# emrullahArkun/tinycarlo

Measured on AMD Instinct MI355X. Metric: env-steps/sec (whole node), higher is better.
Workload: dtype f64; 1 GPU; cfg3: 4096 envs/GPU, simple_layout map, 64x64 'classes' obs, with camera laneline raster; envs_per_gpu=4096, steps_per_launch=128, entry_point=tc_step_multi, observations=every step's frame stored to its own row of a [128, N, ...] rollout buffer, preroll_steps=1024, calls_prepared=True, actions=v~U(0.3,1) s~U(-1,1) maneuver~U{0..3}/64 steps, on device, autoreset=True, spawn=host queue (reference seed parity), resets_since_queue_top_up=18375, max_respawns_of_one_env_since_top_up=11, spawn_queue_len=64, max_segments_per_frame=49, frames_sampled=196608, on_road_term=False, lds_bytes_per_env=9760

## Files before the change

### tinycarlo_amd/csrc/k_camera.h

```cpp
#ifndef K_CAMERA_H
#define K_CAMERA_H

#include "k_common.h"
#include "tc_clip.h"
#include "tc_cull.h"
#include "tc_pack.h"
#include "tc_device.h"

template <int K>
struct MapCache {
  double2 nd[K];
  int2 ed[K];
};

template <int K>
__device__ inline void cache_nodes(MapCache<K>& c, const DevMap& m, int base, int end, int tid) {
#pragma unroll
  for (int k = 0; k < K; k++) {
    const int i = base + k * TC_NT + tid;
    c.nd[k] = i < end ? m.nodes[i] : make_double2(0.0, 0.0);
  }
}
template <int K>
__device__ inline void cache_nodes_from(MapCache<K>& c, const double2* nodes, int base, int end, int tid) {
// ... 385 lines not shown
        }
      }
    }
  }
  __syncthreads();
  cam_chain_replay(Px, Py, Pz, flg, bit, tz, list, *cnt, 0.0, false, tid);
  __syncthreads();
}

struct FramePose {
  double x, y, cth, sth;
};

#define TC_POSE_ROW 16
#define TC_POSE_EMPTY 0xFFFFFFFFFFFFFFFFull
#define TC_FRAME_SKIPPED (-2)
__device__ __forceinline__ void cam_pose12(const KArgs& a, int cam_row, const FramePose& fp, double* pose) {
  double Ec[12];
  if (a.cam_E) {
#pragma unroll
    for (int i = 0; i < 12; i++) Ec[i] = a.cam_E[(size_t)cam_row * 12 + i];
  } else {
    const __attribute__((address_space(4))) double* ee = (const __attribute__((address_space(4))) double*)(unsigned long long)a.cam.E;
#pragma unroll
    for (int i = 0; i < 12; i++) Ec[i] = ee[i];
  }
  const double cth = fp.cth, sth = fp.sth;
  double R[16] = {cth, -sth, 0, 0, sth, cth, 0, 0, 0, 0, 1, 0, 0, 0, 0, 1};
  double Tm[16] = {1, 0, 0, -fp.x, 0, 1, 0, -fp.y, 0, 0, 1, 0, 0, 0, 0, 1};
  double car3d[16];
  d_matmul<4, 4, 4>(R, Tm, car3d);
  d_matmul<3, 4, 4>(Ec, car3d, pose);
}

#ifdef TC_ABLATE
__device__ unsigned long long tc_cull_counts[2];
#endif
__device__ __forceinline__ bool cam_cull(const KArgs& a, const double* pose) {
  typedef const __attribute__((address_space(4))) double* DConst;
  typedef const __attribute__((address_space(4))) int* IConst;
  typedef const __attribute__((address_space(4))) unsigned int* UConst;
  static_assert(offsetof(TcCullHead, margin) == 32 && offsetof(TcCullHead, nx) == 48 && offsetof(TcCullHead, n_special) == 56 &&
                    offsetof(TcCullHead, special) == 64 && TC_CULL_HEAD_BYTES % 4 == 0,
                "the fields are read by offset below");
  const DConst hd = (DConst)(unsigned long long)a.cull_tab;
  const IConst hi = (IConst)(unsigned long long)a.cull_tab;
  TcCullHead h;
  h.x0 = hd[0];
  h.y0 = hd[1];
  h.inv = hd[2];
  h.cell = hd[3];
  h.margin = hd[4];
  h.nx = hi[12];
  h.ny = hi[13];
  h.n_special = hi[14];
  int cell[TC_CULL_NC];
  unsigned int word[TC_CULL_NC];
#pragma unroll
  for (int i = 0; i < TC_CULL_NC; i++) {
    double wx, wy;
    tc_cull_world(pose, a.cull.c[i], &wx, &wy);
    cell[i] = uni_i(tc_cull_cell(h, wx, wy, a.cull.r[i]));
    word[i] = ((UConst)(unsigned long long)a.cull_tab)[(TC_CULL_HEAD_BYTES + (cell[i] > 0 ? cell[i] : 0)) >> 2];
  }
  bool empty = true;
#pragma unroll
  for (int i = 0; i < TC_CULL_NC; i++) {
    const int q = (int)((word[i] >> (8 * (cell[i] & 3))) & 255u);
    empty = empty && (cell[i] == TC_CULL_CELL_CLEAR || (cell[i] >= 0 && tc_cull_free(h, q, a.cull.r[i])));
  }
// ... 1 lines not shown
    const double mr = a.cull.max_range;
    for (int i = 0; i < h.n_special; i++) {
      const double z = __builtin_fma(pose[9], hd[9 + 2 * i], __builtin_fma(pose[8], hd[8 + 2 * i], pose[11]));
      empty = empty && tc_fabs(z + mr) >= TC_CULL_GUARD;
    }
  }
#ifdef TC_ABLATE
  if (threadIdx.x == 0) {
    atomicAdd(&tc_cull_counts[0], 1ull);
    if (empty) atomicAdd(&tc_cull_counts[1], 1ull);
  }
#endif
  return empty;
}

template <int K, bool LEAN = false>
__device__ __forceinline__ void cam_body(const KArgs& a, unsigned char* smem, int env, int cam_row, const double* pose_in, MapCache<K>& mc,
                                         const bool mc_loaded, const int tid, const int seg_row, int& nseg_out,
                                         unsigned int& used_out, const bool store_n = true) {
  unsigned int my_layers = 0;
  const DevMap& m = a.m;
  const int nwin_n = (m.total_nodes + TC_NT * K - 1) / (TC_NT * K), nwin_e = (m.total_edges + TC_NT * K - 1) / (TC_NT * K);
  const bool single = a.n_grp == 1 && !a.cam_nodes && a.grp_layer[0] == 0 && a.grp_layer[1] == m.C && nwin_n <= 1 && nwin_e <= 1;
  double pose[12];
#pragma unroll
  for (int i = 0; i < 12; i++) pose[i] = uni_d(pose_in[i]);
  if (a.frame_cull && cam_cull(a, pose)) {
    nseg_out = 0;
    used_out = 0;
    if (store_n && tid == 0) a.seg_n[(size_t)seg_row * a.N + env] = 0;
    return;
  }
  if (single && !mc_loaded) {
    cache_nodes(mc, m, 0, m.total_nodes, tid);
    cache_edges(mc, m, 0, m.total_edges, 0, tid);
  }
  double* Px = (double*)(smem + a.lds.off_p);
  double* Py = Px + a.cap_nodes;
  double* Pz = Py + a.cap_nodes;
  unsigned char* flg = smem + a.lds.off_flg;
  int* list = (int*)(smem + a.lds.off_list);
  int* cnt = (int*)(smem + a.lds.off_cnt);
  const DevCam& cam = a.cam;
  double Kc[9];
  if constexpr (LEAN) {
  } else if (a.cam_K) {
#pragma unroll
    for (int i = 0; i < 9; i++) Kc[i] = a.cam_K[(size_t)cam_row * 9 + i];
  } else {
    const __attribute__((address_space(4))) double* kk = (const __attribute__((address_space(4))) double*)(unsigned long long)cam.K;
#pragma unroll
    for (int i = 0; i < 9; i++) Kc[i] = kk[i];
  }
  int* seg_cnt = cnt + 5;
  const size_t seg_slot = (size_t)seg_row * a.N + env;
  int* segg = a.seg_g + seg_slot * a.seg_cap * 5;
  int nseg = 0;
  for (int g = 0; g < a.n_grp; g++) {
    const int l0 = a.grp_l0[g], l1 = a.grp_l1[g];
    const int gn0 = a.grp_n0[g], ge0 = a.grp_e0[g];
    const int nn = a.grp_n0[g + 1] - gn0, ne = a.grp_e0[g + 1] - ge0;
    const int nwn = (nn + TC_NT * K - 1) / (TC_NT * K), nwe = (ne + TC_NT * K - 1) / (TC_NT * K);
    const bool one = nwn <= 1 && nwe <= 1;
    const bool reload = !one;
    if (one && !single) {
      if (a.cam_nodes) {
        cache_nodes_from(mc, a.cam_nodes, gn0, gn0 + nn, tid);
        cache_edges_from(mc, a.cam_edges_g, ge0, ge0 + ne, gn0, tid);
      } else {
        cache_nodes(mc, m, gn0, gn0 + nn, tid);
        cache_edges(mc, m, ge0, ge0 + ne, gn0, tid);
      }
// ... 106 lines not shown
```

### tinycarlo_amd/csrc/k_common.h

```cpp
#ifndef K_COMMON_H
#define K_COMMON_H

#include <hip/hip_runtime.h>

#include "../../include/tinycarlo_hip.h"
#include "k_probe.h"
#include "tc_cull.h"
#include "tc_device.h"

#if defined(TC_PART) && defined(TC_DEV_FAST)
#error "the development builds are one translation unit"
#endif
#if defined(TC_PART) && TC_PART > 0
#define TC_PLAIN_KERNEL static
#else
#define TC_PLAIN_KERNEL
#endif

#define TC_PROF_RING 64
#define TC_RING_SLOTS 3
#define MODE_STEP 0
#define MODE_RESET 1
#define MODE_RENDER 2

// ... 75 lines not shown
  int* term_counters;
  int n_grp;
  int grp_layer[TC_MAX_GROUPS + 1];
  int grp_n0[TC_MAX_GROUPS + 1], grp_e0[TC_MAX_GROUPS + 1];
  int grp_l0[TC_MAX_GROUPS], grp_l1[TC_MAX_GROUPS];
  const double2* cam_nodes;
  const int2* cam_edges_g;
  int cap_nodes;
  const int* spawn_tab;
  int spawn_n;
  unsigned long long spawn_seed;
  unsigned int dbg;
  int seg_lds_off, seg_lds_cap;
  int clip_merge;
  int frame_cull;
  const unsigned char* cull_tab;
  TcCullCover cull;
};

__device__ __forceinline__ double d_readlane(double v, int l) {
  const int lo = __builtin_amdgcn_readlane(__double2loint(v), l);
  const int hi = __builtin_amdgcn_readlane(__double2hiint(v), l);
  return __hiloint2double(hi, lo);
}

__device__ __forceinline__ int uni_i(int v) { return __builtin_amdgcn_readfirstlane(v); }
__device__ __forceinline__ double uni_d(double v) {
  const int lo = __builtin_amdgcn_readfirstlane(__double2loint(v));
  const int hi = __builtin_amdgcn_readfirstlane(__double2hiint(v));
  return __hiloint2double(hi, lo);
// ... 56 lines not shown
```

### tinycarlo_amd/csrc/k_env.h

```cpp
#ifndef K_ENV_H
#define K_ENV_H

#include "k_camera.h"
#include "k_raster.h"
#include "k_sim.h"

struct StepArgs {
  KArgs a;
  RArgs r;
  MultiArgs ma;
  int mode, cdtype;
  unsigned int flags;
  const void* car_control;
  const int* maneuver;
  const int* spawn_nodes;
  const unsigned char* mask;
  const int* env_order;
  CarRows cr;
  EpArgs ep;
  CtrlArgs ct;
  CamBank cb;
  DriveArgs dr;
};

// ... 52 lines not shown
    MapCache<K> mc = {};
    FramePose fp;
    int cam_row;
    const bool need_b = k == nsteps - 1 || (sa.flags & TC_FI_INFO_EVERY) != 0;
    sim_body<K, FEAT>(sa.a, smem, env, sa.mode, (const char*)sa.car_control + row0 * 2 * esz, sa.cdtype, sa.maneuver + row0,
                         sa.spawn_nodes, sa.mask, sa.flags, roll_at(sa.ma.roll, row0, sa.a.m.C), tid, mc, fp, cam_row, need_b,
                         need_b || (CAM && sa.ma.cam_here), sa.cr, sa.ep, sa.ct, sa.cb, sa.dr);
    if (sa.ma.pose_rows) {
      double pose[12];
      cam_pose12(sa.a, cam_row, fp, pose);
      if (tid == 0) {
        double2* o = (double2*)(step_args().ma.pose_rows + (row0 + env) * TC_POSE_ROW);
#pragma unroll
        for (int i = 0; i < 6; i++) o[i] = make_double2(pose[2 * i], pose[2 * i + 1]);
        if (sa.flags & TC_FI_CAM_BANK) ((long long*)o)[12] = cam_row;
      }
    }
    if (CAM && sa.ma.cam_here) {
      if (wants_frame(sa)) {
        int nseg;
        unsigned int used;
        double pose[12];
        cam_pose12(sa.a, cam_row, fp, pose);
        cam_body<K>(sa.a, smem, env, cam_row, pose, mc, sa.mode != MODE_RENDER, tid, seg_row, nseg, used);
      }
      else if (tid == 0)
        step_args().a.seg_n[(size_t)seg_row * sa.a.N + env] = 0;
    }
    lds_sync();
  }
// ... 19 lines not shown
```

### tinycarlo_amd/csrc/k_envg.h

```cpp
#ifndef K_ENVG_H
#define K_ENVG_H

#include "k_env.h"

#define TC_EL 8
#ifndef TC_ENVG_NT
#define TC_ENVG_NT 256
#endif
#ifndef TC_ENVG_PRIO
#define TC_ENVG_PRIO 3
#endif
struct GroupLds {
  double dist[TC_MAX_LAYERS];
  int cnt[TC_MAX_TERMS];
};

typedef const __attribute__((address_space(3))) double* LdsDouble;
template <unsigned FEAT>
__device__ __forceinline__ void envg_kernel_body() {
  constexpr bool PER = (FEAT & TC_FEAT_CAR) != 0, EP = (FEAT & TC_FEAT_EP) != 0, CTRL = (FEAT & TC_FEAT_CTRL) != 0;
  __shared__ GroupLds glds[TC_ENVG_NT / TC_EL];
  extern __shared__ __align__(16) unsigned char gsm[];
  __builtin_amdgcn_s_setprio(TC_ENVG_PRIO);
  const StepArgs& s0 = step_args();
// ... 172 lines not shown
    if (sa.ma.pose_rows) {
      FramePose fp;
      fp.x = s.x;
      fp.y = s.y;
      fp.cth = have_trig ? s.cth : tc_cos(-s.theta);
      fp.sth = have_trig ? -s.sth : tc_sin(-s.theta);
      double pose[12];
      cam_pose12(sa.a, cam_row, fp, pose);
      if (live && sub == 0) {
        if (sa.ma.resident) {
          unsigned long long* o = (unsigned long long*)(sa.ma.pose_rows + (row0 + env) * TC_POSE_ROW);
#pragma unroll
          for (int i = 0; i < 12; i++)
            __hip_atomic_store(o + i, (unsigned long long)__double_as_longlong(pose[i]), __ATOMIC_RELAXED, __HIP_MEMORY_SCOPE_AGENT);
          if (bank) __hip_atomic_store(o + 12, (unsigned long long)(unsigned int)cam_row, __ATOMIC_RELAXED, __HIP_MEMORY_SCOPE_AGENT);
        } else {
          double2* o = (double2*)(sa.ma.pose_rows + (row0 + env) * TC_POSE_ROW);
#pragma unroll
          for (int i = 0; i < 6; i++) o[i] = make_double2(pose[2 * i], pose[2 * i + 1]);
          if (bank) ((long long*)o)[12] = cam_row;
        }
      }
    }
    if (track) {
      if (fat_lds) {
        trunc = d_find_local_path<TC_EL>(m, fl, s, track_man, status, pinfo, sub);
      } else {
        const FatGlobal fg = {m.lp_fat, m.lp_nodes};
        trunc = d_find_local_path<TC_EL>(m, fg, s, track_man, status, pinfo, sub);
      }
    }
    TSTAMP(27);
    const bool have_info = !fresh && s.lp_len >= 2;
    cte = 0;
    he = 0;
// ... 210 lines not shown
```

### tinycarlo_amd/csrc/k_frame.h

```cpp
#ifndef K_FRAME_H
#define K_FRAME_H

#include "k_camera.h"
#include "k_env.h"
#include "k_raster.h"
#include "k_sim.h"

struct FrameArgs {
  KArgs a;
  RArgs r;
  const double* pose_rows;
  const int* order;
  int gate;
  int bank;
  int recover_rows;
  unsigned int* abort_word;
  unsigned int* resident;
  long long gate_ticks;
  int gate_test;
};
typedef const __attribute__((address_space(4))) FrameArgs* FrameArgsConst;
__device__ __forceinline__ const FrameArgs& frame_args() {
  unsigned long long p = (unsigned long long)__builtin_amdgcn_kernarg_segment_ptr();
  asm volatile("" : "+s"(p));
  return *(const FrameArgs*)(FrameArgsConst)p;
}
__device__ __forceinline__ bool frame_pose(const size_t slot0, const int env, const int row, const bool wait, double* pose, int& cam_row) {
  const FrameArgs& fa = frame_args();
  const int tid = threadIdx.x;
  const int gate = fa.gate, bank = fa.bank;
  const int np = bank ? 13 : 12;
  cam_row = env;
  if (gate) {
    unsigned long long* prow = (unsigned long long*)(fa.pose_rows + (slot0 + env) * TC_POSE_ROW);
    unsigned long long v = 0;
    bool give_up = wait && fa.gate == 1 && fa.gate_test > 0 && (row + env) % fa.gate_test == 0;
    long long t0 = 0;
    while (!give_up) {
      v = tid < np ? __hip_atomic_load(prow + tid, __ATOMIC_RELAXED, __HIP_MEMORY_SCOPE_AGENT) : 0ull;
      if (__ballot(v == TC_POSE_EMPTY) == 0 || fa.gate == 2 || !wait) break;
      const long long now = wall_clock64();
      if (t0 == 0) t0 = now;
      if (now - t0 > fa.gate_ticks || __hip_atomic_load(fa.abort_word, __ATOMIC_RELAXED, __HIP_MEMORY_SCOPE_AGENT) != 0u)
        give_up = true;
      else
        __builtin_amdgcn_s_sleep(8);
    }
    if (give_up) {
      if (tid == 0) {
        if (t0 != 0) __hip_atomic_store(fa.abort_word, 1u, __ATOMIC_RELAXED, __HIP_MEMORY_SCOPE_AGENT);
        fa.a.seg_n[slot0 + env] = TC_FRAME_SKIPPED;
      }
      return false;
    }
    const unsigned int vlo = (unsigned int)v, vhi = (unsigned int)(v >> 32);
#pragma unroll
    for (int i = 0; i < 12; i++) {
      const unsigned long long q = (unsigned long long)(unsigned int)__builtin_amdgcn_readlane((int)vlo, i) |
                                   ((unsigned long long)(unsigned int)__builtin_amdgcn_readlane((int)vhi, i) << 32);
      pose[i] = __longlong_as_double((long long)q);
    }
    if (bank) {
      const unsigned int idx = (unsigned int)__builtin_amdgcn_readlane((int)vlo, 12);
      cam_row = (int)(idx < (unsigned int)bank ? idx : (unsigned int)bank - 1u);
    }
  } else {
    const __attribute__((address_space(4))) double* pr =
        (const __attribute__((address_space(4))) double*)(unsigned long long)(fa.pose_rows + (slot0 + env) * TC_POSE_ROW);
#pragma unroll
    for (int i = 0; i < 12; i++) pose[i] = pr[i];
    if (bank) {
      const unsigned int idx = ((const __attribute__((address_space(4))) unsigned int*)(unsigned long long)pr)[24];
      cam_row = (int)(idx < (unsigned int)bank ? idx : (unsigned int)bank - 1u);
    }
  }
  return true;
}

#ifndef TC_FRAME_WAVES_K5
#define TC_FRAME_WAVES_K5 5
#endif
#define TC_FRAME_WAVES(K, RBT) ((K) <= 5 ? ((RBT) == 32 ? TC_FRAME_WAVES_K5 : 4) : (K) <= 9 ? 3 : 2)
#define TC_FRAME_LEAN(K, RBT) ((K) <= 5 && (RBT) == 32)
template <int K, bool THICK, int FMT, bool HOT, int RBT, bool ONE_BAND = false>
__device__ __forceinline__ void frame_one(unsigned char* smem, const int env, const int rowy) {
  const int tid = threadIdx.x;
  int nseg;
  unsigned int used;
  {
    const FrameArgs& fa = frame_args();
    const int row = fa.r.seg_row0 + rowy;
    const size_t slot0 = (size_t)row * fa.a.N;
    double pose[12];
    int cam_row;
    if (!frame_pose(slot0, env, row, true, pose, cam_row)) return;
    MapCache<K> mc;
    TSTAMP_CLEAR();
    TSTAMP(3);
    TSTAMP_REAL(30);
    cam_body<K, TC_FRAME_LEAN(K, RBT)>(fa.a, smem, env, cam_row, pose, mc, false, tid, row, nseg, used, false);
  }
  const FrameArgs& fr = frame_args();
  const size_t slot0 = (size_t)(fr.r.seg_row0 + rowy) * fr.a.N;
  if (__builtin_expect(nseg > fr.a.seg_lds_cap, 0)) {
    if (HOT) {
      lds_sync();
      const LdsIntPtr sl = (LdsIntPtr)(smem + fr.a.seg_lds_off);
      int* sg = fr.a.seg_g + (slot0 + env) * fr.a.seg_cap * 5;
      for (int i = tid; i < 5 * fr.a.seg_lds_cap; i += TC_NT) sg[i] = sl[i];
    }
    __syncthreads();
  } else {
    lds_sync();
  }
  raster_body<THICK, FMT, HOT, RBT, TC_FRAME_LEAN(K, RBT), ONE_BAND>(fr.r, smem, env, fr.r.obs + (size_t)rowy * fr.r.obs_row_stride, tid, slot0, nseg, used,
                                           fr.r.noise_row0 + rowy);
  {
    const FrameArgs& fe = frame_args();
    const size_t slot = (size_t)(fe.r.seg_row0 + rowy) * fe.a.N + env;
    if (tid == 0) fe.a.seg_n[slot] = nseg;
    if (fe.gate && tid < (fe.bank ? 13 : 12))
      __hip_atomic_store((unsigned long long*)(fe.pose_rows + slot * TC_POSE_ROW) + tid, TC_POSE_EMPTY, __ATOMIC_RELAXED,
                         __HIP_MEMORY_SCOPE_AGENT);
  }
  TSTAMP_DUMP(env);
}

template <int K, bool THICK, int FMT, int RBT = RB_OF_K(K)>
__global__ __launch_bounds__(TC_NT, TC_FRAME_WAVES(K, RBT)) void tc_frame_kernel(FrameArgs fa_unused) {
  extern __shared__ __align__(16) unsigned char smem[];
  const FrameArgs& fa = frame_args();
  if ((int)blockIdx.x >= fa.a.N) return;
  const int env = fa.order ? uni_i(((const __attribute__((address_space(4))) int*)(unsigned long long)fa.order)[blockIdx.x])
                           : fa.a.env0 + (int)blockIdx.x;
  frame_one<K, THICK, FMT, true, RBT, TC_FRAME_LEAN(K, RBT)>(smem, env, (int)blockIdx.y);
}
// ... 103 lines not shown
```

### tinycarlo_amd/csrc/tc_cull.h

```cpp
#ifndef TC_CULL_H
#define TC_CULL_H
#include "tc_trig.h"

#ifndef TC_CULL_NC
#define TC_CULL_NC 2
#endif
#define TC_CULL_MAX_SPECIAL 16
#define TC_CULL_SLACK 1e-4
#define TC_CULL_GUARD 1e-6
#define TC_CULL_MAX_COORD 1e4
#define TC_CULL_MAX_CELLS (1 << 18)

struct TcCullHead {
  double x0, y0, inv, cell;
  double margin;
  double lmax;
  int nx, ny;
  int n_special, pad;
  double special[TC_CULL_MAX_SPECIAL][2];
};
#define TC_CULL_HEAD_BYTES 320
static_assert(sizeof(TcCullHead) <= TC_CULL_HEAD_BYTES, "the cells start TC_CULL_HEAD_BYTES into the buffer");

struct TcCullCover {
// ... 25 lines not shown
    const double z = __builtin_fma(pose[9], h.special[i][1], __builtin_fma(pose[8], h.special[i][0], pose[11]));
    ok &= tc_fabs(z + max_range) >= TC_CULL_GUARD;
  }
  return ok;
}
TC_HD int tc_cull_empty(const TcCullHead& h, const unsigned char* cells, const TcCullCover& cv, const double* pose) {
  if (!cv.on || h.nx <= 0) return 0;
  for (int i = 0; i < TC_CULL_NC; i++) {
    double wx, wy;
    tc_cull_world(pose, cv.c[i], &wx, &wy);
    const int cell = tc_cull_cell(h, wx, wy, cv.r[i]);
    if (cell == TC_CULL_CELL_MAYBE) return 0;
    if (cell >= 0 && !tc_cull_free(h, cells[cell], cv.r[i])) return 0;
  }
  return tc_cull_guard(h, pose, cv.max_range);
}

#include <math.h>
#include <vector>

static inline double tc_cull_seg_dist(double px, double py, double ax, double ay, double bx, double by) {
  const double ex = bx - ax, ey = by - ay, l2 = ex * ex + ey * ey;
  double t = l2 > 0 ? ((px - ax) * ex + (py - ay) * ey) / l2 : 0.0;
  t = t < 0 ? 0 : (t > 1 ? 1 : t);
  const double dx = px - (ax + t * ex), dy = py - (ay + t * ey);
  return sqrt(dx * dx + dy * dy);
}

static inline void tc_cull_plan(const double* nodes, int n_nodes, const int* edges, int n_edges, double cell, double margin,
                                std::vector<unsigned char>& out) {
// ... 213 lines not shown
```

### tinycarlo_amd/csrc/tinycarlo_hip.hip

```cpp
#include <hip/hip_runtime.h>
#include <math.h>
#include <stdio.h>
#include <stdlib.h>
#include <string.h>

#include <string>
#include <type_traits>
#include <vector>

#include "../../include/tinycarlo_hip.h"
#include "tc_device.h"
#include "tc_rng.h"
#include "tc_ctrl.h"
#include "tc_clip.h"
#include "tc_cull.h"

#include "k_probe.h"
#include "k_common.h"
#include "k_feat.h"
#include "k_collect.h"
#include "k_history.h"
#include "k_camera.h"
#include "k_sim.h"
#include "k_raster.h"
// ... 103 lines not shown
  if (feat & TC_FEAT_CTRL)
    return lift([](auto kc, auto t, auto f, auto ft) -> step_kern_t { return tc_drive_step_kernel<StepKRb<kc>::K, t, f, StepKRb<kc>::RB, ft>; },
                Kcodes{kcode}, Thicks{thick}, Fmts{fmt}, DriveFeats{feat});
  return lift([](auto kc, auto t, auto f, auto ft) -> step_kern_t { return tc_step_kernel<StepKRb<kc>::K, t, f, StepKRb<kc>::RB, ft>; },
              Kcodes{kcode}, Thicks{thick}, Fmts{fmt}, Feats{feat});
}
static step_kern_t env_kernel_of(int kv, bool cam, unsigned feat) {
  if (feat & TC_FEAT_CTRL)
    return lift([](auto k, auto c, auto ft) -> step_kern_t { return tc_drive_env_kernel<k, c, ft>; }, Kvars{kv}, Bools{cam}, DriveFeats{feat});
  return lift([](auto k, auto c, auto ft) -> step_kern_t { return tc_env_kernel<k, c, ft>; }, Kvars{kv}, Bools{cam}, Feats{feat});
}
static step_kern_t envg_kernel_of(unsigned feat) {
  if (feat & TC_FEAT_CTRL) return lift([](auto ft) -> step_kern_t { return tc_drive_envg_kernel<ft>; }, DriveFeats{feat});
  return lift([](auto ft) -> step_kern_t { return tc_envg_kernel<ft>; }, Feats{feat});
}
static frame_kern_t frame_kernel_of(int kcode, bool thick, int fmt, bool recover, bool banded) {
  return lift(
      [](auto kc, auto t, auto f, auto rec, auto bd) -> frame_kern_t {
        constexpr int K = FrameKRb<kc>::K, RB = FrameKRb<kc>::RB;
        if constexpr (rec) return tc_frame_recover_kernel<K, t, f, RB>;
        else if constexpr (bd && TC_FRAME_LEAN(K, RB)) return tc_frame_banded<K, t, f, RB>;
        else return tc_frame_kernel<K, t, f, RB>;
      },
      Kcodes{kcode}, Thicks{thick}, FrameFmts{fmt}, Bools{recover}, Bools{banded});
}
static int frame_k_of(int kcode) {
  return lift([](auto kc) -> int { return FrameKRb<kc>::K; }, Kcodes{kcode});
}
static int frame_rb_of(int kcode) {
  return lift([](auto kc) -> int { return FrameKRb<kc>::RB; }, Kcodes{kcode});
}
static raster_kern_t raster_kernel_of(bool thick, int fmt) {
  return lift([](auto t, auto f) -> raster_kern_t { return tc_raster_kernel<t, f>; }, Thicks{thick}, FrameFmts{fmt});
}

#endif

#if defined(TC_PART) && TC_PART == 1
TC_INST_PART1(template)
// ... 694 lines not shown
    const hipError_t he = rc == TC_OK ? hipFuncSetAttribute(kernel, hipFuncAttributeMaxDynamicSharedMemorySize, bytes) : hipSuccess;
    if (he == hipSuccess) return;
    (void)hipGetLastError();
    set_err(std::string("tc_env_create: cannot raise the dynamic LDS limit of ") + family + " to " + std::to_string(bytes) +
            " bytes: " + hipGetErrorString(he));
    rc = TC_E_HIP;
  };
  int lds = total > e->r_lds ? total : e->r_lds;
  if (e->frame_lds > lds) lds = e->frame_lds;
  if (lds > 48 * 1024)
    for (int kcode : {516, 5, 8, 9})
      for (int t = 0; t < 2; t++)
        for (int fmt : {TC_FMT_CLASSES, TC_FMT_CLASSES_BITS, TC_FMT_RGB}) {
          for (unsigned feat = 0; feat <= (TC_FEAT_CTRL | TC_FEAT_ALL) && fmt != TC_FMT_CLASSES_BITS; feat++)
            raise((const void*)step_kernel_of(kcode, t, fmt, feat), lds, (feat & TC_FEAT_CTRL) ? "tc_drive_step_kernel" : "tc_step_kernel");
          for (int banded = 0; banded < 2; banded++)
            raise((const void*)frame_kernel_of(kcode, t, fmt, false, banded), lds, "tc_frame_kernel");
        }
  const size_t envg_lds = ((size_t)m.total_edges * 48 + 15) / 16 * 16 + (size_t)m.lpN * sizeof(LpNode);
  if (envg_lds > 40 * 1024)
    for (unsigned feat = 0; feat <= (TC_FEAT_CTRL | TC_FEAT_ALL); feat++)
      raise((const void*)envg_kernel_of(feat), (int)(envg_lds < 150 * 1024 ? envg_lds : 150 * 1024),
            (feat & TC_FEAT_CTRL) ? "tc_drive_envg_kernel" : "tc_envg_kernel");
  if (e->r_lds > 48 * 1024)
    for (int t = 0; t < 2; t++)
      for (int fmt : {TC_FMT_CLASSES, TC_FMT_CLASSES_BITS, TC_FMT_RGB}) raise((const void*)raster_kernel_of(t, fmt), e->r_lds, "tc_raster_kernel");
  if (total > 48 * 1024) {
    static const int kvs[4] = {5, 8, 9, 13};
    for (int i = 0; i < 64; i++)
      raise((const void*)env_kernel_of(kvs[i & 3], (i & 4) == 0, (unsigned)i >> 3), total, (i >> 5) ? "tc_drive_env_kernel" : "tc_env_kernel");
  }
  return rc;
// ... 30 lines not shown
  if (hipGetDevice(&dev) == hipSuccess && hipGetDeviceProperties(&prop, dev) == hipSuccess) e->order_g = prop.multiProcessorCount * 4;
  if (e->tune.order_every > 0 && e->order_g > 0 && N % e->order_g == 0 && N / e->order_g <= 4 && N / e->order_g >= 2) {
    std::vector<int> ident((size_t)N);
    for (int i = 0; i < N; i++) ident[(size_t)i] = i;
    DevPtr<int> o;
    if (o.alloc((size_t)N) == hipSuccess && hipMemcpy(o, ident.data(), (size_t)N * sizeof(int), hipMemcpyHostToDevice) == hipSuccess)
      e->env_order = std::move(o);
    else
      (void)hipGetLastError();
  }
}

static void cover_cull(tc_env* e) {
  tc_cull_cover(e->k.cam.E, e->k.cam.K, e->k.cam.W, e->k.cam.H, e->k.cam.max_range, e->cull_head, &e->k.cull);
  e->k.frame_cull = e->tune.frame_cull && e->k.cull_tab && e->k.cull.on && !e->k.cam_E;
}
static int plan_cull(tc_env* e) {
  const tc_map* map = e->map;
  std::vector<unsigned char> tab;
  tc_cull_plan(map->h_nodes.empty() ? nullptr : &map->h_nodes[0].x, (int)map->h_nodes.size(),
               map->h_edges_g.empty() ? nullptr : &map->h_edges_g[0].x, (int)map->h_edges_g.size(), 0.02, 1.0, tab);
  memcpy(&e->cull_head, tab.data(), sizeof(e->cull_head));
  if (e->cull_head.nx > 0) {
    HIP_TRY(e->cull_tab.alloc(tab.size()));
    HIP_TRY(hipMemcpy(e->cull_tab, tab.data(), tab.size(), hipMemcpyHostToDevice));
    e->k.cull_tab = e->cull_tab;
  }
  cover_cull(e);
  return TC_OK;
}
// ... 824 lines not shown
  sa.cb = e->cb;
  sa.cb.rows = ep_rows && e->cb.index && e->cb.rows ? e->cb.rows + r0 : nullptr;
  if (c.roll) sa.ma.roll = rollout_at(*c.roll, r0, (size_t)e->obs_bytes, (size_t)e->k.m.C);
  sa.mode = c.mode;
  sa.cdtype = c.cdtype;
  sa.dr = e->dr;
  sa.dr.man_rows = ep_rows && e->dr.man_rows ? e->dr.man_rows + r0 : nullptr;
  sa.dr.noise_rows = ep_rows && e->dr.noise_rows ? e->dr.noise_rows + r0 : nullptr;
  sa.flags = (c.flags & ~(TC_FI_CAM_BANK | TC_FI_DRIVE | TC_FI_INFO_EVERY)) | (e->cb.index ? TC_FI_CAM_BANK : 0u) |
             (e->dr.tab ? e->drive_flags : 0u) | (c.plan.info_every ? TC_FI_INFO_EVERY : 0u);
  sa.car_control = c.cc ? (const char*)c.cc + r0 * 2 * (c.cdtype == TC_F32 ? 4 : 8) : nullptr;
  sa.maneuver = c.man ? c.man + r0 : nullptr;
  sa.spawn_nodes = c.spawn;
  sa.mask = c.mask;
  return sa;
}

static FrameArgs frame_args_of(const tc_env* e, uint32_t flags, const RArgs& r, bool streamed) {
  FrameArgs fa;
  memset(&fa, 0, sizeof(fa));
  fa.a = e->k;
  fa.a.dbg = flags;
  fa.a.env0 = 0;
  const ScratchRows& s = streamed ? e->streamed : e->ring;
  fa.a.seg_g = s.seg_g;
  fa.a.seg_n = s.seg_n;
  fa.r = r;
  fa.pose_rows = s.pose;
  fa.a.lds.off_p = e->fl.off_p;
  fa.a.lds.off_flg = e->fl.off_flg;
// ... 60 lines not shown
    HIP_TRY(hipEventRecord(e->sim_ev, main));
    HIP_TRY(hipStreamWaitEvent(fs, e->start_ev, 0));
    const int* order;
    rc = frame_order_of(e, 0, fs, true, &order);
    if (rc != TC_OK) return rc;
    RArgs r = make_rargs(e, e->streamed.seg_g, e->streamed.seg_n, e->k.seg_cap, nullptr, c.flags, 0, sa.ma.roll.obs, c.mode == MODE_STEP);
    r.seg_row0 = 0;
    r.noise_row0 = c0;
    r.obs_row_stride = (long long)N * (long long)e->obs_bytes;
    FrameArgs fa = frame_args_of(e, c.flags, r, true);
    fa.order = order;
    hipLaunchKernelGGL(tc_gate_kernel, dim3(1), dim3(64), 0, fs, (const unsigned int*)e->st_words, envg_grid(N), 10 * e->tune.gate_ticks);
    HIP_TRY(hipGetLastError());
    if (c.prof && si == 0) HIP_TRY(hipEventRecord(e->ev[3][c.slot], fs));
    fa.gate = 1;
    hipLaunchKernelGGL(frame_kernel_of(e->kframe, c.thick, c.fmt, false, fa.r.cam.n_bands > 1), dim3(N, cn), dim3(TC_NT), e->frame_lds, fs, fa);
    HIP_TRY(hipGetLastError());
    HIP_TRY(hipStreamWaitEvent(fs, e->sim_ev, 0));
    fa.gate = 2;
    fa.recover_rows = cn;
    fa.order = nullptr;
    hipLaunchKernelGGL(frame_kernel_of(e->kframe, c.thick, c.fmt, true, fa.r.cam.n_bands > 1), dim3(N), dim3(TC_NT), e->frame_lds, fs, fa);
    HIP_TRY(hipGetLastError());
    HIP_TRY(hipEventRecord(e->slot_ev[0], fs));
    if (e->frame_order[0]) e->cost_row[0] = e->streamed.seg_n + (size_t)(cn - 1) * N;
    const int keep = cn < 3 * 16 ? cn : 3 * 16;
    e->draw_rows[0][0] = cn - keep;
    e->draw_rows[0][1] = keep;
    e->draw_n = 1;
  }
  HIP_TRY(hipEventRecord(e->frames_ev, fs));
  HIP_TRY(hipStreamWaitEvent(main, e->frames_ev, 0));
  return TC_OK;
}

static int launch_chunked(tc_env* e, const Call& c) {
  const int N = e->k.N, nsteps = c.nsteps;
// ... 36 lines not shown
      HIP_TRY(hipEventRecord(e->sim_ev, main));
      HIP_TRY(hipStreamWaitEvent(fs, e->sim_ev, 0));
      used_fs[fsi] = true;
    }
    if (c.prof && first_frames && piped) HIP_TRY(hipEventRecord(e->ev[3][c.slot], fs));
    first_frames = false;
    RArgs r = make_rargs(e, e->ring.seg_g, e->ring.seg_n, e->k.seg_cap, nullptr, c.flags, 0, all ? sa.ma.roll.obs : nullptr, c.mode == MODE_STEP);
    r.seg_row0 = (int)rb + (all ? 0 : cn - 1);
    r.noise_row0 = all ? c0 : nsteps - 1;
    r.obs_row_stride = all ? (long long)N * (long long)e->obs_bytes : 0;
    const int rows = all ? cn : 1;
    if (frames) {
      FrameArgs fa = frame_args_of(e, c.flags, r, false);
      int rc = frame_order_of(e, fsi, fs, rows >= 8 || ci < 2, &fa.order);
      if (rc != TC_OK) return rc;
      hipLaunchKernelGGL(frame_kernel_of(e->kframe, c.thick, c.fmt, false, fa.r.cam.n_bands > 1), dim3(N, rows), dim3(TC_NT), e->frame_lds, fs, fa);
      if (e->frame_order[fsi]) e->cost_row[fsi] = e->ring.seg_n + ((size_t)r.seg_row0 + (size_t)rows - 1) * N;
    } else {
      hipLaunchKernelGGL(raster_kernel_of(c.thick, c.fmt), dim3(N, rows), dim3(TC_NT), e->r_lds, fs, r);
    }
    HIP_TRY(hipGetLastError());
    if (piped) HIP_TRY(hipEventRecord(e->slot_ev[rslot], fs));
    {
      const int w = e->draw_n < TC_RING_SLOTS ? e->draw_n++ : (memmove(e->draw_rows[0], e->draw_rows[1], sizeof(int) * 2 * (TC_RING_SLOTS - 1)), TC_RING_SLOTS - 1);
      e->draw_rows[w][0] = r.seg_row0;
      e->draw_rows[w][1] = rows;
    }
  }
  if (used_fs[0]) {
    HIP_TRY(hipEventRecord(e->frames_ev, e->frame_stream));
    HIP_TRY(hipStreamWaitEvent(main, e->frames_ev, 0));
// ... 195 lines not shown
                           : (drive ? "tc_drive_env_kernel" : "tc_env_kernel"));
  return TC_OK;
}

extern "C" int tc_env_frame_lds_info(const tc_env* e, int32_t* lds_bytes, int32_t* head_entries, int32_t* workgroups_per_cu,
                                     int32_t* bits_offset) {
  if (!e) return TC_E_INVALID;
  if (lds_bytes) *lds_bytes = e->frame_lds;
  if (head_entries) *head_entries = e->fl.head_cap;
  if (bits_offset) *bits_offset = e->fl.r_off_bits;
  if (workgroups_per_cu) {
    *workgroups_per_cu = 0;
    if (e->kvar != 13) {
      const DevCam& c = e->k.cam;
      int n = 0;
      HIP_TRY(hipOccupancyMaxActiveBlocksPerMultiprocessor(&n, (const void*)frame_kernel_of(e->kframe, c.thickness > 1, c.format, false, c.n_bands > 1), TC_NT,
                                                           (size_t)e->frame_lds));
      *workgroups_per_cu = n;
    }
  }
  return TC_OK;
}

extern "C" int tc_env_frame_bands(const tc_env* e, int32_t* n_bands, int32_t* band_rows) {
  if (!e) return TC_E_INVALID;
  if (n_bands) *n_bands = e->k.cam.n_bands;
  if (band_rows) *band_rows = e->k.cam.band_rows;
  return TC_OK;
}

extern "C" int tc_render_segments(tc_env* e, const int32_t* segments, const int32_t* counts, int32_t capacity,
// ... 218 lines not shown
```

Measured before the change: 182.4 million env-steps/s.

## Compute frame-cull verdict in step kernel and specialize single-group frame path

```diff
diff --git a/tinycarlo_amd/csrc/k_camera.h b/tinycarlo_amd/csrc/k_camera.h
--- a/tinycarlo_amd/csrc/k_camera.h
+++ b/tinycarlo_amd/csrc/k_camera.h
@@ -423,6 +423,8 @@
 
 #define TC_POSE_ROW 16
 #define TC_POSE_EMPTY 0xFFFFFFFFFFFFFFFFull
+static_assert(TC_CULL_ROW_DRAW != TC_POSE_EMPTY && TC_CULL_ROW_CULLED != TC_POSE_EMPTY && TC_CULL_ROW_ENTRY == 13 && TC_CULL_ROW_ENTRY < TC_POSE_ROW,
+              "a verdict is never read as 'not written yet'");
 #define TC_FRAME_SKIPPED (-2)
 __device__ __forceinline__ void cam_pose12(const KArgs& a, int cam_row, const FramePose& fp, double* pose) {
   double Ec[12];
@@ -445,16 +447,14 @@
 #ifdef TC_ABLATE
 __device__ unsigned long long tc_cull_counts[2];
 #endif
-__device__ __forceinline__ bool cam_cull(const KArgs& a, const double* pose) {
+__device__ __forceinline__ void cam_cull_head(const KArgs& a, TcCullHead& h) {
   typedef const __attribute__((address_space(4))) double* DConst;
   typedef const __attribute__((address_space(4))) int* IConst;
-  typedef const __attribute__((address_space(4))) unsigned int* UConst;
   static_assert(offsetof(TcCullHead, margin) == 32 && offsetof(TcCullHead, nx) == 48 && offsetof(TcCullHead, n_special) == 56 &&
                     offsetof(TcCullHead, special) == 64 && TC_CULL_HEAD_BYTES % 4 == 0,
                 "the fields are read by offset below");
   const DConst hd = (DConst)(unsigned long long)a.cull_tab;
   const IConst hi = (IConst)(unsigned long long)a.cull_tab;
-  TcCullHead h;
   h.x0 = hd[0];
   h.y0 = hd[1];
   h.inv = hd[2];
@@ -463,6 +463,13 @@
   h.nx = hi[12];
   h.ny = hi[13];
   h.n_special = hi[14];
+}
+__device__ __forceinline__ bool cam_cull(const KArgs& a, const double* pose) {
+  typedef const __attribute__((address_space(4))) double* DConst;
+  typedef const __attribute__((address_space(4))) unsigned int* UConst;
+  const DConst hd = (DConst)(unsigned long long)a.cull_tab;
+  TcCullHead h;
+  cam_cull_head(a, h);
   int cell[TC_CULL_NC];
   unsigned int word[TC_CULL_NC];
 #pragma unroll
@@ -494,10 +501,46 @@
   return empty;
 }
 
-template <int K, bool LEAN = false>
+__device__ __forceinline__ unsigned long long cam_cull_row(const KArgs& a, const double* pose) {
+  typedef const __attribute__((address_space(4))) double* DConst;
+  const DConst hd = (DConst)(unsigned long long)a.cull_tab;
+  TcCullHead h;
+  cam_cull_head(a, h);
+  bool empty = true;
+#pragma unroll
+  for (int i = 0; i < TC_CULL_NC; i++) {
+    double wx, wy;
+    tc_cull_world(pose, a.cull.c[i], &wx, &wy);
+    const int cell = tc_cull_cell(h, wx, wy, a.cull.r[i]);
+    const int q = (int)a.cull_tab[TC_CULL_HEAD_BYTES + (cell > 0 ? cell : 0)];
+    empty = empty && (cell == TC_CULL_CELL_CLEAR || (cell >= 0 && tc_cull_free(h, q, a.cull.r[i])));
+  }
+  if (empty) {
+    const double mr = a.cull.max_range;
+    for (int i = 0; i < h.n_special; i++) {
+      const double z = __builtin_fma(pose[9], hd[9 + 2 * i], __builtin_fma(pose[8], hd[8 + 2 * i], pose[11]));
+      empty = empty && tc_fabs(z + mr) >= TC_CULL_GUARD;
+    }
+  }
+  return tc_cull_row_encode(empty);
+}
+
+template <int K, bool LEAN = false, bool ROW = false, bool ONE_GROUP = false>
 __device__ __forceinline__ void cam_body(const KArgs& a, unsigned char* smem, int env, int cam_row, const double* pose_in, MapCache<K>& mc,
                                          const bool mc_loaded, const int tid, const int seg_row, int& nseg_out,
-                                         unsigned int& used_out, const bool store_n = true) {
+                                         unsigned int& used_out, const bool store_n = true, const bool row_culled = false) {
+#ifdef TC_ABLATE
+  if (ROW && a.cull_rows && threadIdx.x == 0) {
+    atomicAdd(&tc_cull_counts[0], 1ull);
+    if (row_culled) atomicAdd(&tc_cull_counts[1], 1ull);
+  }
+#endif
+  if (ROW && row_culled) {
+    nseg_out = 0;
+    used_out = 0;
+    if (store_n && tid == 0) a.seg_n[(size_t)seg_row * a.N + env] = 0;
+    return;
+  }
   unsigned int my_layers = 0;
   const DevMap& m = a.m;
   const int nwin_n = (m.total_nodes + TC_NT * K - 1) / (TC_NT * K), nwin_e = (m.total_edges + TC_NT * K - 1) / (TC_NT * K);
@@ -505,7 +548,7 @@
   double pose[12];
 #pragma unroll
   for (int i = 0; i < 12; i++) pose[i] = uni_d(pose_in[i]);
-  if (a.frame_cull && cam_cull(a, pose)) {
+  if (!ROW && a.frame_cull && cam_cull(a, pose)) {
     nseg_out = 0;
     used_out = 0;
     if (store_n && tid == 0) a.seg_n[(size_t)seg_row * a.N + env] = 0;
@@ -536,6 +579,21 @@
   const size_t seg_slot = (size_t)seg_row * a.N + env;
   int* segg = a.seg_g + seg_slot * a.seg_cap * 5;
   int nseg = 0;
+  if constexpr (ONE_GROUP) {
+    const int gn0 = a.grp_n0[0], ge0 = a.grp_e0[0];
+    const int nn = a.grp_n0[1] - gn0, ne = a.grp_e0[1] - ge0;
+    if (!single) {
+      if (a.cam_nodes) {
+        cache_nodes_from(mc, a.cam_nodes, gn0, gn0 + nn, tid);
+        cache_edges_from(mc, a.cam_edges_g, ge0, ge0 + ne, gn0, tid);
+      } else {
+        cache_nodes(mc, m, gn0, gn0 + nn, tid);
+        cache_edges(mc, m, ge0, ge0 + ne, gn0, tid);
+      }
+    }
+    cam_group_regs<K, LEAN>(a, mc, pose, Kc, cam_row, a.grp_l0[0], a.grp_l1[0], ge0, nn, ne, Px, Py, Pz, flg, list, segg,
+                            (LdsIntPtr)(smem + a.seg_lds_off), nseg, my_layers, env, tid);
+  } else
   for (int g = 0; g < a.n_grp; g++) {
     const int l0 = a.grp_l0[g], l1 = a.grp_l1[g];
     const int gn0 = a.grp_n0[g], ge0 = a.grp_e0[g];
diff --git a/tinycarlo_amd/csrc/k_common.h b/tinycarlo_amd/csrc/k_common.h
--- a/tinycarlo_amd/csrc/k_common.h
+++ b/tinycarlo_amd/csrc/k_common.h
@@ -113,6 +113,7 @@
   int seg_lds_off, seg_lds_cap;
   int clip_merge;
   int frame_cull;
+  int cull_rows;
   const unsigned char* cull_tab;
   TcCullCover cull;
 };
diff --git a/tinycarlo_amd/csrc/k_env.h b/tinycarlo_amd/csrc/k_env.h
--- a/tinycarlo_amd/csrc/k_env.h
+++ b/tinycarlo_amd/csrc/k_env.h
@@ -90,6 +90,7 @@
 #pragma unroll
         for (int i = 0; i < 6; i++) o[i] = make_double2(pose[2 * i], pose[2 * i + 1]);
         if (sa.flags & TC_FI_CAM_BANK) ((long long*)o)[12] = cam_row;
+        if (sa.a.cull_rows) ((unsigned long long*)o)[TC_CULL_ROW_ENTRY] = cam_cull_row(step_args().a, pose);
       }
     }
     if (CAM && sa.ma.cam_here) {
diff --git a/tinycarlo_amd/csrc/k_envg.h b/tinycarlo_amd/csrc/k_envg.h
--- a/tinycarlo_amd/csrc/k_envg.h
+++ b/tinycarlo_amd/csrc/k_envg.h
@@ -210,11 +210,14 @@
           for (int i = 0; i < 12; i++)
             __hip_atomic_store(o + i, (unsigned long long)__double_as_longlong(pose[i]), __ATOMIC_RELAXED, __HIP_MEMORY_SCOPE_AGENT);
           if (bank) __hip_atomic_store(o + 12, (unsigned long long)(unsigned int)cam_row, __ATOMIC_RELAXED, __HIP_MEMORY_SCOPE_AGENT);
+          if (sa.a.cull_rows)
+            __hip_atomic_store(o + TC_CULL_ROW_ENTRY, cam_cull_row(sa.a, pose), __ATOMIC_RELAXED, __HIP_MEMORY_SCOPE_AGENT);
         } else {
           double2* o = (double2*)(sa.ma.pose_rows + (row0 + env) * TC_POSE_ROW);
 #pragma unroll
           for (int i = 0; i < 6; i++) o[i] = make_double2(pose[2 * i], pose[2 * i + 1]);
           if (bank) ((long long*)o)[12] = cam_row;
+          if (sa.a.cull_rows) ((unsigned long long*)o)[TC_CULL_ROW_ENTRY] = cam_cull_row(sa.a, pose);
         }
       }
     }
diff --git a/tinycarlo_amd/csrc/k_frame.h b/tinycarlo_amd/csrc/k_frame.h
--- a/tinycarlo_amd/csrc/k_frame.h
+++ b/tinycarlo_amd/csrc/k_frame.h
@@ -25,19 +25,23 @@
   asm volatile("" : "+s"(p));
   return *(const FrameArgs*)(FrameArgsConst)p;
 }
-__device__ __forceinline__ bool frame_pose(const size_t slot0, const int env, const int row, const bool wait, double* pose, int& cam_row) {
+__device__ __forceinline__ bool frame_pose(const size_t slot0, const int env, const int row, const bool wait, double* pose, int& cam_row,
+                                           bool& culled) {
   const FrameArgs& fa = frame_args();
   const int tid = threadIdx.x;
   const int gate = fa.gate, bank = fa.bank;
-  const int np = bank ? 13 : 12;
+  const bool verdict = fa.a.cull_rows != 0;
   cam_row = env;
+  culled = false;
   if (gate) {
     unsigned long long* prow = (unsigned long long*)(fa.pose_rows + (slot0 + env) * TC_POSE_ROW);
     unsigned long long v = 0;
     bool give_up = wait && fa.gate == 1 && fa.gate_test > 0 && (row + env) % fa.gate_test == 0;
     long long t0 = 0;
     while (!give_up) {
-      v = tid < np ? __hip_atomic_load(prow + tid, __ATOMIC_RELAXED, __HIP_MEMORY_SCOPE_AGENT) : 0ull;
+      v = (tid < 12 || (tid == 12 && bank) || (tid == TC_CULL_ROW_ENTRY && verdict))
+              ? __hip_atomic_load(prow + tid, __ATOMIC_RELAXED, __HIP_MEMORY_SCOPE_AGENT)
+              : 0ull;
       if (__ballot(v == TC_POSE_EMPTY) == 0 || fa.gate == 2 || !wait) break;
       const long long now = wall_clock64();
       if (t0 == 0) t0 = now;
@@ -53,6 +57,11 @@
       }
       return false;
     }
+    static_assert(TC_CULL_ROW_ENTRY > 12 && TC_CULL_ROW_ENTRY < TC_POSE_ROW && TC_CULL_ROW_ENTRY < TC_NT, "a lane and a row entry of its own");
+    if (__ballot(tid == TC_CULL_ROW_ENTRY && tc_cull_row_decode(v)) != 0) {
+      culled = true;
+      return true;
+    }
     const unsigned int vlo = (unsigned int)v, vhi = (unsigned int)(v >> 32);
 #pragma unroll
     for (int i = 0; i < 12; i++) {
@@ -67,6 +76,10 @@
   } else {
     const __attribute__((address_space(4))) double* pr =
         (const __attribute__((address_space(4))) double*)(unsigned long long)(fa.pose_rows + (slot0 + env) * TC_POSE_ROW);
+    if (verdict && tc_cull_row_decode(((const __attribute__((address_space(4))) unsigned long long*)(unsigned long long)pr)[TC_CULL_ROW_ENTRY])) {
+      culled = true;
+      return true;
+    }
 #pragma unroll
     for (int i = 0; i < 12; i++) pose[i] = pr[i];
     if (bank) {
@@ -82,7 +95,7 @@
 #endif
 #define TC_FRAME_WAVES(K, RBT) ((K) <= 5 ? ((RBT) == 32 ? TC_FRAME_WAVES_K5 : 4) : (K) <= 9 ? 3 : 2)
 #define TC_FRAME_LEAN(K, RBT) ((K) <= 5 && (RBT) == 32)
-template <int K, bool THICK, int FMT, bool HOT, int RBT, bool ONE_BAND = false>
+template <int K, bool THICK, int FMT, bool HOT, int RBT, bool ONE = false>
 __device__ __forceinline__ void frame_one(unsigned char* smem, const int env, const int rowy) {
   const int tid = threadIdx.x;
   int nseg;
@@ -93,12 +106,13 @@
     const size_t slot0 = (size_t)row * fa.a.N;
     double pose[12];
     int cam_row;
-    if (!frame_pose(slot0, env, row, true, pose, cam_row)) return;
+    bool culled;
+    if (!frame_pose(slot0, env, row, true, pose, cam_row, culled)) return;
     MapCache<K> mc;
     TSTAMP_CLEAR();
     TSTAMP(3);
     TSTAMP_REAL(30);
-    cam_body<K, TC_FRAME_LEAN(K, RBT)>(fa.a, smem, env, cam_row, pose, mc, false, tid, row, nseg, used, false);
+    cam_body<K, TC_FRAME_LEAN(K, RBT), true, ONE>(fa.a, smem, env, cam_row, pose, mc, false, tid, row, nseg, used, false, culled);
   }
   const FrameArgs& fr = frame_args();
   const size_t slot0 = (size_t)(fr.r.seg_row0 + rowy) * fr.a.N;
@@ -113,13 +127,13 @@
   } else {
     lds_sync();
   }
-  raster_body<THICK, FMT, HOT, RBT, TC_FRAME_LEAN(K, RBT), ONE_BAND>(fr.r, smem, env, fr.r.obs + (size_t)rowy * fr.r.obs_row_stride, tid, slot0, nseg, used,
+  raster_body<THICK, FMT, HOT, RBT, TC_FRAME_LEAN(K, RBT), ONE>(fr.r, smem, env, fr.r.obs + (size_t)rowy * fr.r.obs_row_stride, tid, slot0, nseg, used,
                                            fr.r.noise_row0 + rowy);
   {
     const FrameArgs& fe = frame_args();
     const size_t slot = (size_t)(fe.r.seg_row0 + rowy) * fe.a.N + env;
     if (tid == 0) fe.a.seg_n[slot] = nseg;
-    if (fe.gate && tid < (fe.bank ? 13 : 12))
+    if (fe.gate && (tid < 12 || (tid == 12 && fe.bank) || (tid == TC_CULL_ROW_ENTRY && fe.a.cull_rows)))
       __hip_atomic_store((unsigned long long*)(fe.pose_rows + slot * TC_POSE_ROW) + tid, TC_POSE_EMPTY, __ATOMIC_RELAXED,
                          __HIP_MEMORY_SCOPE_AGENT);
   }
diff --git a/tinycarlo_amd/csrc/tc_cull.h b/tinycarlo_amd/csrc/tc_cull.h
--- a/tinycarlo_amd/csrc/tc_cull.h
+++ b/tinycarlo_amd/csrc/tc_cull.h
@@ -63,6 +63,15 @@
     if (cell >= 0 && !tc_cull_free(h, cells[cell], cv.r[i])) return 0;
   }
   return tc_cull_guard(h, pose, cv.max_range);
+}
+
+#define TC_CULL_ROW_ENTRY 13
+#define TC_CULL_ROW_DRAW 0ull
+#define TC_CULL_ROW_CULLED 1ull
+TC_HD unsigned long long tc_cull_row_encode(int empty) { return empty ? TC_CULL_ROW_CULLED : TC_CULL_ROW_DRAW; }
+TC_HD int tc_cull_row_decode(unsigned long long w) { return w == TC_CULL_ROW_CULLED; }
+TC_HD unsigned long long tc_cull_row_verdict(const TcCullHead& h, const unsigned char* cells, const TcCullCover& cv, const double* pose) {
+  return tc_cull_row_encode(tc_cull_empty(h, cells, cv, pose));
 }
 
 #include <math.h>
diff --git a/tinycarlo_amd/csrc/tinycarlo_hip.hip b/tinycarlo_amd/csrc/tinycarlo_hip.hip
--- a/tinycarlo_amd/csrc/tinycarlo_hip.hip
+++ b/tinycarlo_amd/csrc/tinycarlo_hip.hip
@@ -141,7 +141,7 @@
   if (feat & TC_FEAT_CTRL) return lift([](auto ft) -> step_kern_t { return tc_drive_envg_kernel<ft>; }, DriveFeats{feat});
   return lift([](auto ft) -> step_kern_t { return tc_envg_kernel<ft>; }, Feats{feat});
 }
-static frame_kern_t frame_kernel_of(int kcode, bool thick, int fmt, bool recover, bool banded) {
+static frame_kern_t frame_kernel_of(int kcode, bool thick, int fmt, bool recover, bool looped) {
   return lift(
       [](auto kc, auto t, auto f, auto rec, auto bd) -> frame_kern_t {
         constexpr int K = FrameKRb<kc>::K, RB = FrameKRb<kc>::RB;
@@ -149,7 +149,7 @@
         else if constexpr (bd && TC_FRAME_LEAN(K, RB)) return tc_frame_banded<K, t, f, RB>;
         else return tc_frame_kernel<K, t, f, RB>;
       },
-      Kcodes{kcode}, Thicks{thick}, FrameFmts{fmt}, Bools{recover}, Bools{banded});
+      Kcodes{kcode}, Thicks{thick}, FrameFmts{fmt}, Bools{recover}, Bools{looped});
 }
 static int frame_k_of(int kcode) {
   return lift([](auto kc) -> int { return FrameKRb<kc>::K; }, Kcodes{kcode});
@@ -874,8 +874,8 @@
         for (int fmt : {TC_FMT_CLASSES, TC_FMT_CLASSES_BITS, TC_FMT_RGB}) {
           for (unsigned feat = 0; feat <= (TC_FEAT_CTRL | TC_FEAT_ALL) && fmt != TC_FMT_CLASSES_BITS; feat++)
             raise((const void*)step_kernel_of(kcode, t, fmt, feat), lds, (feat & TC_FEAT_CTRL) ? "tc_drive_step_kernel" : "tc_step_kernel");
-          for (int banded = 0; banded < 2; banded++)
-            raise((const void*)frame_kernel_of(kcode, t, fmt, false, banded), lds, "tc_frame_kernel");
+          for (int looped = 0; looped < 2; looped++)
+            raise((const void*)frame_kernel_of(kcode, t, fmt, false, looped), lds, "tc_frame_kernel");
         }
   const size_t envg_lds = ((size_t)m.total_edges * 48 + 15) / 16 * 16 + (size_t)m.lpN * sizeof(LpNode);
   if (envg_lds > 40 * 1024)
@@ -936,6 +936,7 @@
 static void cover_cull(tc_env* e) {
   tc_cull_cover(e->k.cam.E, e->k.cam.K, e->k.cam.W, e->k.cam.H, e->k.cam.max_range, e->cull_head, &e->k.cull);
   e->k.frame_cull = e->tune.frame_cull && e->k.cull_tab && e->k.cull.on && !e->k.cam_E;
+  e->k.cull_rows = e->k.frame_cull;
 }
 static int plan_cull(tc_env* e) {
   const tc_map* map = e->map;
@@ -1790,6 +1791,11 @@
   sa.spawn_nodes = c.spawn;
   sa.mask = c.mask;
   return sa;
+}
+
+static bool frame_looped(const tc_env* e) {
+  const int kf = frame_k_of(e->kframe);
+  return e->k.cam.n_bands > 1 || e->k.n_grp != 1 || e->k.grp_n0[1] - e->k.grp_n0[0] > kf * TC_NT || e->k.grp_e0[1] - e->k.grp_e0[0] > kf * TC_NT;
 }
 
 static FrameArgs frame_args_of(const tc_env* e, uint32_t flags, const RArgs& r, bool streamed) {
@@ -1880,13 +1886,13 @@
     HIP_TRY(hipGetLastError());
     if (c.prof && si == 0) HIP_TRY(hipEventRecord(e->ev[3][c.slot], fs));
     fa.gate = 1;
-    hipLaunchKernelGGL(frame_kernel_of(e->kframe, c.thick, c.fmt, false, fa.r.cam.n_bands > 1), dim3(N, cn), dim3(TC_NT), e->frame_lds, fs, fa);
+    hipLaunchKernelGGL(frame_kernel_of(e->kframe, c.thick, c.fmt, false, frame_looped(e)), dim3(N, cn), dim3(TC_NT), e->frame_lds, fs, fa);
     HIP_TRY(hipGetLastError());
     HIP_TRY(hipStreamWaitEvent(fs, e->sim_ev, 0));
     fa.gate = 2;
     fa.recover_rows = cn;
     fa.order = nullptr;
-    hipLaunchKernelGGL(frame_kernel_of(e->kframe, c.thick, c.fmt, true, fa.r.cam.n_bands > 1), dim3(N), dim3(TC_NT), e->frame_lds, fs, fa);
+    hipLaunchKernelGGL(frame_kernel_of(e->kframe, c.thick, c.fmt, true, frame_looped(e)), dim3(N), dim3(TC_NT), e->frame_lds, fs, fa);
     HIP_TRY(hipGetLastError());
     HIP_TRY(hipEventRecord(e->slot_ev[0], fs));
     if (e->frame_order[0]) e->cost_row[0] = e->streamed.seg_n + (size_t)(cn - 1) * N;
@@ -1953,7 +1959,7 @@
       FrameArgs fa = frame_args_of(e, c.flags, r, false);
       int rc = frame_order_of(e, fsi, fs, rows >= 8 || ci < 2, &fa.order);
       if (rc != TC_OK) return rc;
-      hipLaunchKernelGGL(frame_kernel_of(e->kframe, c.thick, c.fmt, false, fa.r.cam.n_bands > 1), dim3(N, rows), dim3(TC_NT), e->frame_lds, fs, fa);
+      hipLaunchKernelGGL(frame_kernel_of(e->kframe, c.thick, c.fmt, false, frame_looped(e)), dim3(N, rows), dim3(TC_NT), e->frame_lds, fs, fa);
       if (e->frame_order[fsi]) e->cost_row[fsi] = e->ring.seg_n + ((size_t)r.seg_row0 + (size_t)rows - 1) * N;
     } else {
       hipLaunchKernelGGL(raster_kernel_of(c.thick, c.fmt), dim3(N, rows), dim3(TC_NT), e->r_lds, fs, r);
@@ -2179,7 +2185,7 @@
     if (e->kvar != 13) {
       const DevCam& c = e->k.cam;
       int n = 0;
-      HIP_TRY(hipOccupancyMaxActiveBlocksPerMultiprocessor(&n, (const void*)frame_kernel_of(e->kframe, c.thickness > 1, c.format, false, c.n_bands > 1), TC_NT,
+      HIP_TRY(hipOccupancyMaxActiveBlocksPerMultiprocessor(&n, (const void*)frame_kernel_of(e->kframe, c.thickness > 1, c.format, false, frame_looped(e)), TC_NT,
                                                            (size_t)e->frame_lds));
       *workgroups_per_cu = n;
     }
```

After: 185.8 million env-steps/s (median of 6 runs). 1.02x the previous value.
